# xinxu27/turbo_decoder_cuda

Measured on AMD Instinct MI355X. Metric: decoded info Mbit/s @ K=6144, 8 iter, Eb/N0=1.0 dB; BER match vs CPU log_map, higher is better.
Workload: dtype f64

## Files before the change

include/turbo_mi355x.h:

```cpp
#ifndef TURBO_MI355X_H
#define TURBO_MI355X_H

#include <stdint.h>

#ifdef __cplusplus
extern "C" {
#endif

#define TD_ABI_VERSION 1

enum td_status {
    TD_OK = 0,
    TD_EINVAL = 1,
    TD_ENOMEM = 2,
    TD_EHIP = 3,
    TD_ENODEV = 4
};

enum td_algo {
    TD_ALGO_LOGMAP = 0,
    TD_ALGO_MAXLOG = 1
};

enum td_precision {
// ... 15 lines not shown
int td_create(td_handle** out, const td_params* p);
int td_destroy(td_handle* h);
int td_reserve(td_handle* h, int B);

int td_decode_device(td_handle* h, const void* d_llr, int B, uint8_t* d_bits, int all_iters, void* d_le,
                     void* stream);

int td_debug_window_layout(td_handle* h, int run, int run_a, int parts);
typedef struct td_window_params {
    int window;
    int overlap;
    int nii;
    int concurrent;
    double ext_scale;
} td_window_params;
enum td_window_maxstar { TD_WMAXSTAR_FAST = 0, TD_WMAXSTAR_EXACT = 1 };
int td_set_window_maxstar(td_handle* h, int form);
int td_set_window(td_handle* h, const td_window_params* w);

enum td_stop_rule { TD_STOP_NONE = 0, TD_STOP_HDA = 1, TD_STOP_CRC = 2 };
typedef struct td_stop_params {
    int rule;
    int min_iters;
    uint32_t crc_poly;
} td_stop_params;
int td_set_early_stop(td_handle* h, const td_stop_params* s);
int td_set_window_stop(td_handle* h, const td_stop_params* s);
int td_decode_device_stop(td_handle* h, const void* d_llr, int B, uint8_t* d_bits, int all_iters, void* d_le,
                          int32_t* d_iters, void* stream);
int td_decode_host_stop(td_handle* h, const void* llr, int B, int* out, void* le, int* iters_used);
uint32_t td_crc24_host(const uint8_t* bits, int K, uint32_t poly);
int td_crc24_syndromes(int K, uint32_t poly, uint32_t* table );

int td_profile_enable(td_handle* h, int on);
int td_profile_read(td_handle* h, float* demux_ms, float* decode_ms, int* launches);
int td_clock_read(td_handle* h, double* sclk_ghz, double* span_ms);

int td_debug_set_stamps(td_handle* h, void* d_buf);
int td_debug_stamp_slots(void);
int td_debug_placement(td_handle* h, float* ms, int cap, int* pick);
int td_debug_placement_cost(td_handle* h, double* wall_ms, double* held_bytes);
int td_debug_workspace_bytes(td_handle* h, unsigned long long* bytes);
int td_debug_placement_rule(const float* ms, int n);

int td_window_steps(void);

int td_decode_host(td_handle* h, const void* llr, int B, int* out, void* le);

int td_siso_host(td_handle* h, const void* recs, const void* La, int terminated, void* LLR, int L, int B);

int td_synth_seed(td_handle* h, unsigned seed);
int td_synth_seek(td_handle* h, unsigned long long frame);
int td_rand_window(unsigned seed, unsigned long long draws, uint32_t* win);
int td_synth_frames(td_handle* h, double ebn0_db, int B, uint8_t* d_info, double* d_llr, void* stream);

int td_synth_modulation(td_handle* h, int modulation);

int td_modulate(const uint8_t* d_bits, long long nsym, int modulation, double* d_si, double* d_sq, void* stream);
int td_demodulate(const double* d_yi, const double* d_yq, long long nsym, int modulation, double Kf, double* d_llr,
                  void* stream);

int td_count_errors(td_handle* h, const uint8_t* d_bits, int iters, const uint8_t* d_info, int B, int* d_err,
                    void* stream);

const char* td_last_error(void);
int td_device_count(void);
// ... 14 lines not shown
```

turbo_decoder_cuda_amd/_native.py:

```python
from __future__ import annotations

import ctypes as C
import os

PKG = os.path.dirname(os.path.abspath(__file__))
LIB_PATH = os.environ.get("TD_LIB_PATH") or os.path.join(PKG, "libturbo_mi355x.so")

TD_OK, TD_EINVAL, TD_ENOMEM, TD_EHIP, TD_ENODEV = 0, 1, 2, 3, 4
TD_ALGO_LOGMAP, TD_ALGO_MAXLOG = 0, 1
TD_F64, TD_F32 = 0, 1
TD_WMAXSTAR_FAST, TD_WMAXSTAR_EXACT = 0, 1
TD_MAXSTAR_WINDOW_FAST = 2
TD_STOP_NONE, TD_STOP_HDA, TD_STOP_CRC = 0, 1, 2
CRC24A, CRC24B = 0x864CFB, 0x800063

EXPORTS = (
    "td_create", "td_destroy", "td_reserve", "td_decode_device", "td_decode_host", "td_siso_host",
    "td_last_error", "td_device_count", "td_abi_version", "td_maxstar_host_f64", "td_maxstar_host_f32",
    "td_trellis_tables", "td_qpp_table", "td_profile_enable", "td_profile_read", "td_debug_set_stamps",
    "td_debug_stamp_slots", "td_synth_seed", "td_synth_frames", "td_count_errors", "td_rand_window", "td_synth_seek",
    "td_set_window", "td_synth_modulation", "td_modulate", "td_demodulate", "td_debug_placement",
    "td_debug_placement_rule", "td_clock_read", "td_window_steps", "td_debug_placement_cost", "td_debug_window_layout",
    "td_debug_workspace_bytes", "td_set_window_maxstar", "td_set_early_stop", "td_decode_device_stop",
    "td_decode_host_stop", "td_crc24_host", "td_crc24_syndromes", "td_set_window_stop",
)


class TdParams(C.Structure):
    _fields_ = [
        ("K", C.c_int), ("f1", C.c_int), ("f2", C.c_int), ("iterations", C.c_int),
        ("algo", C.c_int), ("precision", C.c_int), ("device", C.c_int),
    ]


class TdWindowParams(C.Structure):
    _fields_ = [("window", C.c_int), ("overlap", C.c_int), ("nii", C.c_int), ("concurrent", C.c_int),
                ("ext_scale", C.c_double)]


class TdStopParams(C.Structure):
    _fields_ = [("rule", C.c_int), ("min_iters", C.c_int), ("crc_poly", C.c_uint32)]


class TurboError(RuntimeError):
    def __init__(self, code: int, msg: str):
        super().__init__(f"turbo_mi355x error {code}: {msg}")
        self.code = code


_lib = None


def lib() -> C.CDLL:
    global _lib
    if _lib is not None:
        return _lib
    if not os.path.exists(LIB_PATH):
# ... 16 lines not shown
    L.td_device_count.restype = I
    L.td_abi_version.restype = I
    L.td_maxstar_host_f64.argtypes = [C.c_double, C.c_double, I]
    L.td_maxstar_host_f64.restype = C.c_double
    L.td_maxstar_host_f32.argtypes = [C.c_float, C.c_float, I]
    L.td_maxstar_host_f32.restype = C.c_float
    L.td_trellis_tables.argtypes = [P, P, P]
    L.td_qpp_table.argtypes = [I, I, I, P]
    L.td_profile_enable.argtypes = [P, I]
    L.td_debug_set_stamps.argtypes = [P, P]
    L.td_debug_stamp_slots.restype = I
    L.td_debug_placement.argtypes = [P, C.POINTER(C.c_float), I, C.POINTER(C.c_int)]
    L.td_debug_placement_rule.argtypes = [C.POINTER(C.c_float), I]
    if hasattr(L, "td_debug_placement_cost"):
        L.td_debug_placement_cost.argtypes = [P, C.POINTER(C.c_double), C.POINTER(C.c_double)]
    L.td_profile_read.argtypes = [P, C.POINTER(C.c_float), C.POINTER(C.c_float), C.POINTER(C.c_int)]
    if hasattr(L, "td_clock_read"):
        L.td_clock_read.argtypes = [P, C.POINTER(C.c_double), C.POINTER(C.c_double)]
    L.td_synth_seed.argtypes = [P, C.c_uint]
    L.td_rand_window.argtypes = [C.c_uint, C.c_ulonglong, P]
    L.td_synth_seek.argtypes = [P, C.c_ulonglong]
    L.td_synth_frames.argtypes = [P, C.c_double, I, P, P, P]
    L.td_count_errors.argtypes = [P, P, I, P, I, P, P]
    L.td_set_window.argtypes = [P, C.POINTER(TdWindowParams)]
    if hasattr(L, "td_set_early_stop"):
        L.td_set_early_stop.argtypes = [P, C.POINTER(TdStopParams)]
        L.td_decode_device_stop.argtypes = [P, P, I, P, I, P, P, P]
        L.td_decode_host_stop.argtypes = [P, P, I, P, P, P]
        L.td_crc24_host.argtypes = [P, I, C.c_uint32]
        L.td_crc24_host.restype = C.c_uint32
        L.td_crc24_syndromes.argtypes = [I, C.c_uint32, P]
    if hasattr(L, "td_set_window_stop"):
        L.td_set_window_stop.argtypes = [P, C.POINTER(TdStopParams)]
    L.td_synth_modulation.argtypes = [P, I]
    L.td_modulate.argtypes = [P, C.c_longlong, I, P, P, P]
    L.td_demodulate.argtypes = [P, P, C.c_longlong, I, C.c_double, P, P]
    _lib = L
    return L


def check(rc: int) -> None:
    if rc != TD_OK:
        raise TurboError(rc, lib().td_last_error().decode(errors="replace"))
```

turbo_decoder_cuda_amd/csrc/td_api.cpp:

```cpp
#include <hip/hip_runtime_api.h>

#include <cmath>
#include <cstdio>
#include <algorithm>
#include <array>
#include <chrono>
#include <cstdlib>
#include <cstring>
#include <string>
#include <vector>

#include "td_crc.h"
#include "td_kernels.h"

#ifndef TD_SYS2_IN_TURBO
#define TD_SYS2_IN_TURBO 1
#endif
#ifndef TD_PLACEMENT_DEFAULT
#define TD_PLACEMENT_DEFAULT 24
#endif
#include "td_tables.h"
#include "turbo_mi355x.h"

namespace {
// ... 34 lines not shown
    unsigned* d_slots = nullptr;
    unsigned long long* d_clk = nullptr;
    bool clk_valid = false;
    void* d_hin = nullptr;
    uint8_t* d_hbits = nullptr;
    void* d_hle = nullptr;
    size_t hin_b = 0, hbits_b = 0, hle_b = 0;
    int32_t* d_hiters = nullptr;
    size_t hiters_b = 0;
    std::vector<uint8_t> h_hbits;
    void* d_ws = nullptr;
    std::vector<float> place_ms;
    int place_pick = -1;
    double place_wall_ms = 0, place_held = 0;
    size_t ws_bytes = 0;
    size_t elem = 8;
    void* stamps = nullptr;
    bool prof = false;
    std::vector<std::array<hipEvent_t, 3>> ev;
    size_t nev = 0;
    uint32_t lfg_win[31] = {};
    uint32_t lfg_win0[31] = {};
    std::vector<uint32_t> lfg_jump;
    bool lfg_seeded = false;
    unsigned long long lfg_frames = 0;
    uint32_t* d_win = nullptr;
    int win_cap = 0;
    int modulation = 1;
    int role_cus = 0;
    int occ3 = 1;
    td::WindowParams wp{0, 0, 0, 0, 1.0, 0};
    int win_run = 0, win_run_a = 0, win_parts = 0;
    int win_exact_table = 0;
    void* d_wws = nullptr;
    size_t wws_bytes = 0;
    td::WindowStreams wstr{};
    td_stop_params stop{TD_STOP_NONE, 1, 0};
    uint32_t* d_crc = nullptr;
    td_stop_params wstop{TD_STOP_NONE, 1, 0};
    bool clk_stopped = false;
    hipEvent_t ws_free = nullptr;
    hipStream_t ws_stream = nullptr;
    bool ws_pending = false;
};

namespace td {

bool build_lane_tables(const Trellis& t, LaneTables& lt)
{
    auto A = [](int l) { return (l & 1) ^ (((l >> 1) & 1) * 2) ^ (((l >> 2) & 1) * 7); };
    auto rotr = [](int s) { return (s >> 1) | ((s & 1) << 2); };
    const int m[3] = {1, 2, 7};
    for (int ph = 0; ph < 3; ++ph)
        for (int l = 0; l < 8; ++l) {
            int s = A(l);
            for (int r = 0; r < ph; ++r) s = rotr(s);
            lt.state[ph][l] = s;
        }
    for (int ph = 0; ph < 3; ++ph) {
        const int nx = (ph + 1) % 3;
        for (int l = 0; l < 8; ++l) {
            const int j = lt.state[nx][l], ps = lt.state[ph][l], pp = lt.state[ph][l ^ m[ph]];
            const int p0 = t.laststat[j][0], p1 = t.laststat[j][1];
            if (!((ps == p0 && pp == p1) || (ps == p1 && pp == p0))) return false;
            const int us = ps == p0 ? 0 : 1;
            const int os = t.nextout[ps][2 * us + 1], op = t.nextout[pp][2 * (1 - us) + 1];
// ... 333 lines not shown
int decode_device_t(td_handle* h, const void* d_llr, int B, uint8_t* d_bits, int all_iters, void* d_le,
                    int32_t* d_iters, hipStream_t st)
{
    const int G = groups_for(B);
    int rc = ensure_ws(h, G);
    if (rc) return rc;
    const Carve c = carve_for(h, G);
    char* ws = static_cast<char*>(h->d_ws);
    td::DecodeParams<T> dp{};
    fill_common(dp, h);
    dp.sys1 = reinterpret_cast<T*>(ws + c.sys1);
    dp.par1 = reinterpret_cast<T*>(ws + c.par1);
    dp.sys2 = reinterpret_cast<T*>(ws + c.sys2);
    dp.par2 = reinterpret_cast<T*>(ws + c.par2);
    dp.ext12 = reinterpret_cast<T*>(ws + c.ext12);
    dp.ext21 = reinterpret_cast<T*>(ws + c.ext21);
    dp.astore = reinterpret_cast<T*>(ws + c.astore);
    dp.tmstore = reinterpret_cast<T*>(ws + c.tmstore);
    dp.llr_out = nullptr;
    dp.pi = h->d_pi;
    dp.pinv = h->d_pinv;
    dp.bits = d_bits;
    dp.le_dump = static_cast<T*>(d_le);
    dp.stamps = static_cast<unsigned long long*>(h->stamps);
    dp.clk = h->d_clk;
    dp.K = h->p.K;
    dp.L = h->p.K + td::kMemory;
    dp.nT = (dp.L + td::window_steps() - 1) / td::window_steps();
    dp.G = G;
    dp.B = B;
    dp.iters = h->p.iterations;
    dp.all_iters = all_iters ? 1 : 0;
    dp.sys2_in_turbo = (TD_SYS2_IN_TURBO && !h->wp.window) ? 1 : 0;
    td::WindowBufs<T> wb{};
    if (h->wp.window) {
        if (!h->wstr.st[1]) return fail(TD_EINVAL, "td_decode_device: the windowed schedule's streams are missing");
        rc = window_bufs<T>(h, dp, wb);
        if (rc) return rc;
    }
    hipStreamCaptureStatus cap = hipStreamCaptureStatusNone;
    TD_HIP(hipStreamIsCapturing(st, &cap));
    const bool capturing = cap != hipStreamCaptureStatusNone;
    if (!capturing) {
        if (!h->ws_free) TD_HIP(hipEventCreateWithFlags(&h->ws_free, hipEventDisableTiming));
        if (h->ws_pending && st != h->ws_stream) TD_HIP(hipStreamWaitEvent(st, h->ws_free, 0));
    }
    hipEvent_t* ev = nullptr;
    if (h->prof && !capturing) {
        if (h->nev == h->ev.size()) {
            std::array<hipEvent_t, 3> tri{};
            for (auto& x : tri) TD_HIP(hipEventCreate(&x));
            h->ev.push_back(tri);
        }
        ev = h->ev[h->nev].data();
        TD_HIP(hipEventRecord(ev[0], st));
    }
    hipError_t e = h->wp.window ? td::launch_window_demux<T>(dp, static_cast<const T*>(d_llr), st)
                                : td::launch_demux<T>(dp, static_cast<const T*>(d_llr), st);
    if (e != hipSuccess) return hip_fail(e, "launch_demux");
    if (ev) TD_HIP(hipEventRecord(ev[1], st));
    const bool wstop = h->wp.window && h->wstop.rule != TD_STOP_NONE;
    if (wstop) {
        const td::StopParams sp{h->wstop.rule, h->wstop.min_iters, h->d_crc, d_iters};
        e = td::launch_window<T>(dp, h->wp, wb, st, h->wstr, &sp);
    } else if (h->wp.window) {
        e = td::launch_window<T>(dp, h->wp, wb, st, h->wstr);
    } else if (h->stop.rule != TD_STOP_NONE) {
        const td::StopParams sp{h->stop.rule, h->stop.min_iters, h->d_crc, d_iters};
        e = td::launch_turbo<T>(dp, st, false, &sp);
    } else {
        e = td::launch_turbo<T>(dp, st);
    }
    if (e == hipSuccess && d_iters && h->stop.rule == TD_STOP_NONE && !wstop)
        e = hipMemsetD32Async(reinterpret_cast<hipDeviceptr_t>(d_iters), h->p.iterations, (size_t)B, st);
    if (e != hipSuccess) return hip_fail(e, h->wp.window ? "launch_window" : "launch_turbo");
    h->clk_valid = !capturing;
    h->clk_stopped = wstop;
    if (ev) {
        TD_HIP(hipEventRecord(ev[2], st));
        ++h->nev;
    }
    if (!capturing) {
        TD_HIP(hipEventRecord(h->ws_free, st));
        h->ws_stream = st;
        h->ws_pending = true;
    }
    return TD_OK;
}

template <typename T>
int siso_host_t(td_handle* h, const void* recs, const void* La, int terminated, void* LLR, int L, int B)
// ... 399 lines not shown
    const int rc = ensure_wstr(h);
    if (rc) return rc;
    h->wp = td::WindowParams{w->window, w->overlap, w->nii ? 1 : 0, w->concurrent ? 1 : 0, w->ext_scale,
                             h->win_run, h->win_run_a, h->win_parts, h->win_exact_table};
    return TD_OK;
}

int td_set_window_maxstar(td_handle* h, int form)
{
    if (!h) return fail(TD_EINVAL, "td_set_window_maxstar: null handle");
    if (form != TD_WMAXSTAR_FAST && form != TD_WMAXSTAR_EXACT)
        return fail(TD_EINVAL, "td_set_window_maxstar: form must be TD_WMAXSTAR_FAST or TD_WMAXSTAR_EXACT");
    h->win_exact_table = form == TD_WMAXSTAR_EXACT ? 1 : 0;
    h->wp.exact_table = h->win_exact_table;
    return TD_OK;
}

int td_debug_window_layout(td_handle* h, int run, int run_a, int parts)
{
    if (!h) return fail(TD_EINVAL, "td_debug_window_layout: null handle");
    if (run < 0 || run_a < 0 || parts < 0 || parts > td::kSwMaxParts)
        return fail(TD_EINVAL, "td_debug_window_layout: run, run_a >= 0 and 0 <= parts <= 4");
    h->win_run = run;
    h->win_run_a = run_a;
    h->win_parts = parts;
    if (h->wp.window) {
        h->wp.run = run;
        h->wp.run_a = run_a;
        h->wp.parts = parts;
    }
    return TD_OK;
}

int td_profile_enable(td_handle* h, int on)
{
    if (!h) return fail(TD_EINVAL, "td_profile_enable: null handle");
    h->prof = on != 0;
    h->nev = 0;
    return TD_OK;
}

int td_profile_read(td_handle* h, float* demux_ms, float* decode_ms, int* launches)
{
    if (!h || !h->prof) return fail(TD_EINVAL, "td_profile_read: profiling not enabled");
    TD_HIP(hipSetDevice(h->p.device));
    double sa = 0, sb = 0;
    for (size_t k = 0; k < h->nev; ++k) {
        float a = 0, b = 0;
        TD_HIP(hipEventSynchronize(h->ev[k][2]));
        TD_HIP(hipEventElapsedTime(&a, h->ev[k][0], h->ev[k][1]));
        TD_HIP(hipEventElapsedTime(&b, h->ev[k][1], h->ev[k][2]));
        sa += a;
        sb += b;
    }
    const int n = (int)h->nev;
    if (demux_ms) *demux_ms = n ? (float)(sa / n) : 0.f;
    if (decode_ms) *decode_ms = n ? (float)(sb / n) : 0.f;
    if (launches) *launches = n;
    h->nev = 0;
    return TD_OK;
}

int td_clock_read(td_handle* h, double* sclk_ghz, double* span_ms)
{
    if (!h) return fail(TD_EINVAL, "td_clock_read: null handle");
    if (!h->clk_valid) return fail(TD_EINVAL, "td_clock_read: the last decode was captured into a graph");
// ... 220 lines not shown
```

turbo_decoder_cuda_amd/csrc/td_kernels.h:

```cpp
#pragma once

#include <hip/hip_runtime_api.h>

#include <cstdint>

#include "td_tables.h"

namespace td {

struct LaneTables {
    int state[3][8];
    int a_sg[3][8], a_sel[3][8];
    int a_pg[3][8], a_psel[3][8];
    int b_sg[3][8], b_sel[3][8];
    int b_pg[3][8], b_psel[3][8];
    int a_j[3][8];
    int a_swap[3][8];
};

bool build_lane_tables(const Trellis& t, LaneTables& lt);

constexpr int kPermPad = 32;
constexpr int kGroupWaves = 4;
constexpr int kCuSlotKeys = 2048;
constexpr int kWindowStepsMax = 15;
constexpr size_t astore_group_elems(int L) { return ((size_t)L + 1) * 64; }
constexpr size_t astore_elems(int G, int L) { return (size_t)G * astore_group_elems(L) + (size_t)2 * kWindowStepsMax * 64; }

template <typename T>
struct DecodeParams {
    T* sys1;
    T* par1;
    T* sys2;
    T* par2;
    T* ext12;
    T* ext21;
    T* astore;
    T* tmstore;
    T* llr_out;
    const int* pi;
    const int* pinv;
    const LutEntry<T>* lut;
    const T* qlut;
    uint8_t* bits;
    T* le_dump;
    unsigned long long* stamps;
    unsigned long long* clk;
    int K, L, nT, G, B, iters, all_iters, algo;
    int role_cus;
    int occ3;
    int sys2_in_turbo;
    unsigned* cu_slots;
    int nextstat[kStates][2];
    int laststat[kStates][2];
    int nextout[kStates][4];
    const LaneTables* lane;
};

struct StopParams {
    int rule;
    int min_iters;
    const uint32_t* crc_tab;
    int* iters_out;
};

template <typename T>
hipError_t launch_demux(const DecodeParams<T>& p, const T* flow, hipStream_t st);
template <typename T>
hipError_t launch_window_demux(const DecodeParams<T>& p, const T* flow, hipStream_t st);
template <typename T>
hipError_t launch_turbo(const DecodeParams<T>& p, hipStream_t st, bool probe = false,
                        const StopParams* stop = nullptr);
template <typename T, int ALGO>
hipError_t launch_turbo4_w12(const DecodeParams<T>& p, hipStream_t st, const StopParams* stop = nullptr);

struct WindowParams {
    int window;
    int overlap;
    int nii;
    int concurrent;
    double ext_scale;
    int run;
    int run_a;
    int parts;
    int exact_table;
};
template <typename T>
struct WindowBufs {
    T* ext12[2];
    T* ext21[2];
    T* nii;
    T* ckpt[2];
    uint8_t* bitsT;
    int* stop_at;
    unsigned* stop_ev;
};
inline int window_subblocks(int L, int W) { return L / W > 0 ? L / W : 1; }
size_t window_ckpt_elems(int B, int L, int W, bool f32);
// ... 36 lines not shown
```

turbo_decoder_cuda_amd/csrc/td_kernels.hip:

```cpp
#include <hip/hip_runtime.h>

#include <cstdint>
#include <type_traits>

#include "td_kernels.h"
#include "td_tables.h"

#ifdef TD_W12_TU
namespace td_w12 {
using namespace ::td;
#else
namespace td {
#endif

#ifndef TD_KW
#define TD_KW 15
#endif
constexpr int kW = TD_KW;
static_assert(kW == 12 || kW == 15, "windows of 12 or 15 steps");
static_assert(kW <= kWindowStepsMax, "the host sizes the alpha scratch's DMA tail for the longest window");
constexpr int kArow0 = kW / 2;
constexpr int kCw = 8;
constexpr int kLanes = 64;
constexpr int kTile = kW * kCw;
static_assert(kW % 3 == 0, "window must be a multiple of the label period");

#ifndef TD_DIAG
#define TD_DIAG 0
#endif
constexpr unsigned kDiagNoAdma = 1;
constexpr unsigned kDiagNoBConvert = 2;
constexpr unsigned kDiagNoFold = 4;
constexpr unsigned kDiagNoBeta = 8;
constexpr unsigned kDiagOcc3Alias = 16;
constexpr unsigned kDiagNoAStore = 32;
constexpr unsigned kDiagFoldNoLut = 64;
constexpr unsigned kDiagSwNoCk = 128;
// ... 281 lines not shown
{
    if (!kFoldSwz<T>) return off;
    return (off & ~7) + blk_off<T>(off & 7, r);
}

__device__ __forceinline__ void wg_sync_lds()
{
    asm volatile("s_waitcnt lgkmcnt(0)\n\ts_barrier" ::: "memory");
}

template <typename T>
struct SisoSrc {
    const T* sys;
    const T* par;
    const T* la;
    int la_cap;
    int la_len;
    int terminated;
};

template <typename T>
struct SisoDst {
    T* ext;
    int ext_mode;
    int ext_len;
    T* llr;
    T* le_dump;
    uint8_t* bits;
    int bits_row;
    int bits_stride;
    int dump_slot;
    int dump_stride;
    T* sys2_out;
};

struct Geom {
    int K, L, nT, B, g, G;
    const int* pi;
    const int* pinv;
};

__device__ __forceinline__ int window_len(const Geom& gm, int t) { return min(kW, gm.L - t * kW); }

template <typename T>
__device__ __forceinline__ void load_elem(const SisoSrc<T>& src, const Geom& gm, int t, int e, T& ys, T& yp, T& la,
                                          bool want_yp)
{
    const int k = e >> 3, c = e & 7;
    const int i = min(t * kW + k, gm.L - 1);
    const size_t off = ((size_t)gm.g * gm.L + i) * kCw + c;
    ys = src.sys[off];
    yp = want_yp ? src.par[off] : (T)0;
    la = src.la[((size_t)gm.g * src.la_cap + min(i, src.la_cap - 1)) * kCw + c];
}

template <typename T>
__device__ __forceinline__ T la_at(const SisoSrc<T>& src, int i, T raw)
{
    return i < src.la_len ? raw : (T)0;
}

template <int N>
__device__ __forceinline__ void vm_wait()
{
    asm volatile("s_waitcnt vmcnt(%0)" ::"n"(N) : "memory");
}
// ... 984 lines not shown
        asm volatile("s_waitcnt lgkmcnt(0)" ::: "memory");
        TD_STAMP(bc);
        TD_ACC(14, b0, bc);
        tile_dma(sm, slot, src, dst, gm, max(min(wa - 3, tl - 3), 0), lane);
        tm_dma(sm, slot, tmstore, gm, wa - 3, lane);
        if constexpr (kAd > 0) alpha_dma<T, ALGO>(sm, astore, gm, wa - 1, lane);
        TD_STAMP(bw);
        vm_wait<2 * kB>();
        TD_STAMP(b1);
        TD_ACC(4, bw, b1);
        wg_sync_lds();
        TD_STAMP(b2);
        TD_ACC(2, b0, b1);
        TD_ACC(3, b1, b2);
    };
    tile_dma(sm, 0, src, dst, gm, max(tl - 3, 0), lane);
    tm_dma(sm, 0, tmstore, gm, tl, lane);
    tile_dma(sm, 1, src, dst, gm, max(tl - 3, 0), lane);
    tm_dma(sm, 1, tmstore, gm, tl - 1, lane);
    tile_dma(sm, 2, src, dst, gm, max(tl - 3, 0), lane);
    tm_dma(sm, 2, tmstore, gm, tl - 2, lane);
    if constexpr (kAd > 0) alpha_dma<T, ALGO>(sm, astore, gm, tl, lane);
    vm_wait<2 * (kF + 1) + kAd>();
    TD_STAMP(p4);
    TD_ACC(12, p3, p4);
    for (int j = 0; j < nB; j += 3) {
        bstep(j, 0);
        if (j + 1 < nB) bstep(j + 1, 1);
        if (j + 2 < nB) bstep(j + 2, 2);
    }
    asm volatile("s_waitcnt vmcnt(0)" ::: "memory");
}

template <typename T, int ALGO, bool STOP = false>
__device__ void siso_wg(Smem<T>& sm, const SisoSrc<T>& src, const SisoDst<T>& dst, const Geom& gm, T* astore,
                        T* tmstore, const LaneTables* lt, int wave, int lane, unsigned long long* st,
                        StopLane* sl = nullptr)
{
    (void)st;
    (void)sl;
    if constexpr (kRoleRemat<T>) touch(lane);
    TD_STAMP(p0);
    const int nT = gm.nT;
    const int tl = nT - 1;
    const int nB = nT + 2;
    T* ga0 = astore + astore_window_off(gm.g, 0, gm.L);
    constexpr size_t aws = (size_t)kW * kLanes;
    T* gtm0 = tmstore + (size_t)gm.g * gm.L * kCw;

    if (wave == 0) {
        const int c = lane >> 3;
        LaneConst<T> lc;
        lane_setup(lt, lane, lc);
        T a = lc.a_init0 ? (T)0 : (T)-kInfty;
        __builtin_amdgcn_s_setprio(kAlphaPrio);
        wg_sync_lds();
        TD_STAMP(p1);
        TD_ACC(11, p0, p1);
        int t0 = 0;
        if constexpr (kAlphaSchedS<T, ALGO>) {
            if (tl >= 2) {
                TD_STAMP(f0);
                a = alpha_window<T, ALGO>(a, 0, kW, sm, lut_col(sm, lane), c, lc, ga0, gtm0, st ? st + 4 : nullptr);
                TD_STAMP(f1);
                wg_sync_lds();
                TD_STAMP(f2);
                TD_ACC(0, f0, f1);
                TD_ACC(1, f1, f2);
// ... 61 lines not shown
    } else if (wave == 2) {
        constexpr int kF = kTileDma<T>;
        auto fstep = [&](int t) {
            TD_STAMP(f0);
            if (t + 1 <= tl) tile_convert(sm, (t + 1) % 3, src, t + 1, lane);
            if (!kFSkip<ALGO> || t + 3 <= tl) {
                tile_dma(sm, t % 3, src, dst, gm, min(t + 3, tl), lane);
                vm_wait<kF>();
            } else {
                vm_wait<0>();
            }
            TD_STAMP(f1);
            wg_sync_lds();
            TD_STAMP(f2);
            TD_ACC(0, f0, f1);
            TD_ACC(1, f1, f2);
        };
        tile_dma(sm, 0, src, dst, gm, 0, lane);
        vm_wait<0>();
        TD_STAMP(p2);
        TD_ACC(13, p0, p2);
        tile_convert(sm, 0, src, 0, lane);
        tile_dma(sm, 1, src, dst, gm, min(1, tl), lane);
        tile_dma(sm, 2, src, dst, gm, min(2, tl), lane);
        vm_wait<kF>();
        wg_sync_lds();
        TD_STAMP(p1);
        TD_ACC(11, p0, p1);
        for (int t = 0; t < nT; ++t) fstep(t);
        if constexpr (kBLoaderWave<ALGO> == 2) {
            bpass_loader<T, ALGO>(sm, src, dst, gm, astore, tmstore, lane, tl, nB, st);
            return;
        }
    } else if (dst.sys2_out) {
        wg_sync_lds();
        TD_STAMP(p1);
        TD_ACC(11, p0, p1);
        const int e = (wave == 1 ? 0 : kLanes) + lane;
        const int ec = min(e, kTile - 1);
        const int k = ec >> 3, c = ec & 7;
        const T* s1 = src.sys + (size_t)gm.g * gm.L * kCw + c;
        T* s2 = dst.sys2_out + (size_t)gm.g * gm.L * kCw + c;
        T v = (T)0;
        int ip = -1;
        for (int t = 0; t < nT; ++t) {
            TD_STAMP(f0);
            const int pi_i = min(max(sm.Wp[t % 3][k][1], 0), gm.K - 1);
            const T nv = s1[(size_t)pi_i * kCw];
            if (ip >= 0) s2[(size_t)ip * kCw] = v;
            const int i = t * kW + k;
            ip = (e < kTile && i < gm.K) ? i : -1;
            v = nv;
            TD_STAMP(f1);
            wg_sync_lds();
            TD_STAMP(f2);
            TD_ACC(0, f0, f1);
            TD_ACC(1, f1, f2);
        }
        if (ip >= 0) s2[(size_t)ip * kCw] = v;
        asm volatile("s_waitcnt vmcnt(0)" ::: "memory");
    } else {
        wg_sync_lds();
        TD_STAMP(p1);
        TD_ACC(11, p0, p1);
        for (int t = 0; t < nT; ++t) {
            TD_STAMP(f0);
// ... 213 lines not shown
__device__ __forceinline__ void wg_release(const WgPos& w, unsigned* slots)
{
    if (w.slot < 4) {
        __syncthreads();
        if (threadIdx.x == 0) atomicAnd(&slots[w.slot_key], ~(1u << w.slot));
    }
}

template <typename T, int ALGO, bool STOP = false>
__device__ __forceinline__ void turbo_decode_body(const DecodeParams<T>& p, const StopParams* sp = nullptr)
{
    (void)sp;
    const WgPos w = wg_pos(p.role_cus, p.cu_slots);
    Smem<T>& sm = *smem<T>();
    const int wave = w.role, lane = w.lane;
    lut_to_lds(p, sm, wave * kLanes + lane);
    if (wave == 1) set_beta_prio<T, ALGO>();
    [[maybe_unused]] StopLane sl{};
    [[maybe_unused]] unsigned long long used = 0;
    [[maybe_unused]] int stop_first = 0;
    if constexpr (STOP) {
        __shared__ unsigned s_stop[kCw];
        if (threadIdx.x < kCw) s_stop[threadIdx.x] = 0;
        sl.rule = sp->rule;
        sl.crc_tab = sp->crc_tab;
        sl.lds = s_stop;
        sl.prev_off = p.all_iters ? -(long long)p.K : 0;
        for (int c = 0; c < kCw; ++c) {
            if (w.g * kCw + c >= p.B) sl.done |= 1u << c;
            used |= (unsigned long long)p.iters << (8 * c);
        }
        stop_first = max(sp->rule == 1 ? 2 : 1, sp->min_iters);
    }
    __syncthreads();

    Geom gm{p.K, p.L, p.nT, p.B, w.g, p.G, p.pi, p.pinv};
    unsigned long long st[kStampSlots] = {};
#ifdef TD_STAMPS
    const unsigned long long k_cyc0 = __builtin_amdgcn_s_memtime(), k_rt0 = __builtin_amdgcn_s_memrealtime();
#endif
    const bool clk = p.clk && blockIdx.x == 0;
    unsigned long long clk_c0 = 0, clk_r0 = 0;
    if (clk) {
        clk_c0 = __builtin_amdgcn_s_memtime();
        clk_r0 = __builtin_amdgcn_s_memrealtime();
    }
    for (int s = 0; s < 2 * p.iters; ++s) {
        const int it = s >> 1, dec = s & 1;
        const bool want_bits = dec == 1 && (STOP || p.all_iters || it == p.iters - 1);
        SisoSrc<T> src{dec ? p.sys2 : p.sys1, dec ? p.par2 : p.par1, dec ? p.ext12 : p.ext21, p.K,
                       (dec == 0 && it == 0) ? 0 : p.K, 1};
        SisoDst<T> dst{dec ? p.ext21 : p.ext12, dec ? 2 : 3, p.K, nullptr, p.le_dump,
                       want_bits ? p.bits : nullptr, p.all_iters ? it : 0, p.all_iters ? p.iters * p.K : p.K,
                       s, p.iters * 2 * p.L, (s == 0 && p.sys2_in_turbo) ? p.sys2 : nullptr};
        TD_STAMP(s0);
        if constexpr (STOP) {
            sl.acc = 0;
            sl.has_prev = it > 0;
        }
        siso_wg<T, ALGO, STOP>(sm, src, dst, gm, p.astore, p.tmstore, p.lane, wave, lane, st, &sl);
        TD_STAMP(s1);
        __syncthreads();
        TD_STAMP(s2);
        TD_ACC(9, s0, s1);
        TD_ACC(10, s1, s2);
        if constexpr (STOP) {
            if (dec == 1 && it + 1 < p.iters) {
                unsigned stop = 0;
                if (it + 1 >= stop_first) {
                    if (sl.rule == 1) {
                        stop = ~sl.lds[0] & 0xffu;
                    } else {
#pragma unroll
                        for (int c = 0; c < kCw; ++c) stop |= (sl.lds[c] == 0 ? 1u : 0u) << c;
                    }
                }
                stop = (unsigned)__builtin_amdgcn_readfirstlane((int)stop) & ~sl.done;
#pragma unroll
                for (int c = 0; c < kCw; ++c)
                    if ((stop >> c) & 1)
                        used = (used & ~(0xffull << (8 * c))) | ((unsigned long long)(it + 1) << (8 * c));
                sl.done |= stop;
                __syncthreads();
                if (threadIdx.x < kCw) sl.lds[threadIdx.x] = 0;
                if (sl.done == 0xffu) break;
            }
        }
// ... 949 lines not shown
    if (e != hipSuccess) return e;
    if (probe)
        hipLaunchKernelGGL((turbo_placement_probe_kernel<T, ALGO>), dim3(p.G), dim3(kWaves * kLanes), wg_lds<T>(), st, p);
    else
        hipLaunchKernelGGL((turbo_decode_kernel<T, ALGO>), dim3(p.G), dim3(kWaves * kLanes), wg_lds<T>(), st, p);
    return hipGetLastError();
}

template <typename T, int ALGO>
hipError_t launch_siso_algo(const DecodeParams<T>& p, const T* la, int terminated, hipStream_t st)
{
    hipError_t e = allow_smem(reinterpret_cast<const void*>(&siso_kernel<T, ALGO>), wg_lds<T>());
    if (e != hipSuccess) return e;
    hipLaunchKernelGGL((siso_kernel<T, ALGO>), dim3(p.G), dim3(kWaves * kLanes), wg_lds<T>(), st, p, la, terminated);
    return hipGetLastError();
}

template <typename T>
hipError_t launch_demux(const DecodeParams<T>& p, const T* flow, hipStream_t st)
{
    const size_t total = (size_t)p.G * p.L * kCw;
    int gblocks = (int)((total + 255) / 256);
    if (gblocks > kDemuxBlocks) gblocks = kDemuxBlocks;
    hipLaunchKernelGGL(demux_kernel<T>, dim3(gblocks), dim3(256), 0, st, p, flow);
    hipError_t e = hipGetLastError();
    if (e != hipSuccess) return e;
    if (p.sys2_in_turbo) return hipSuccess;
    const int bpg = (p.K * kCw + kPermBlock - 1) / kPermBlock;
    const long long pblocks = (long long)((p.G + 7) / 8) * 8 * bpg;
    hipLaunchKernelGGL(demux_perm_kernel<T>, dim3((unsigned)pblocks), dim3(kPermBlock), 0, st, p, bpg);
    return hipGetLastError();
}

template <typename T>
hipError_t launch_turbo(const DecodeParams<T>& p, hipStream_t st, bool probe, const StopParams* stop)
{
    return p.algo == 1 ? launch_turbo_algo<T, 1>(p, st, probe, stop) : launch_turbo_algo<T, 0>(p, st, probe, stop);
}

template <typename T>
hipError_t launch_siso(const DecodeParams<T>& p, const T* recs, const T* la, T* la_ws, int terminated, T* llr,
                       hipStream_t st)
{
    const size_t total = (size_t)p.G * p.L * kCw;
    int gblocks = (int)((total + 255) / 256);
    if (gblocks > kDemuxBlocks) gblocks = kDemuxBlocks;
    hipLaunchKernelGGL(siso_in_kernel<T>, dim3(gblocks), dim3(256), 0, st, p, recs, la, la_ws);
    hipError_t e = p.algo == 1 ? launch_siso_algo<T, 1>(p, la_ws, terminated, st)
                               : launch_siso_algo<T, 0>(p, la_ws, terminated, st);
    if (e != hipSuccess) return e;
    hipLaunchKernelGGL(siso_out_kernel<T>, dim3(gblocks), dim3(256), 0, st, p, llr);
    return hipGetLastError();
}

#if !defined(TD_W12_TU) && !defined(TD_WIN_TU)
template hipError_t launch_demux<double>(const DecodeParams<double>&, const double*, hipStream_t);
template hipError_t launch_demux<float>(const DecodeParams<float>&, const float*, hipStream_t);
template hipError_t launch_turbo<double>(const DecodeParams<double>&, hipStream_t, bool, const StopParams*);
template hipError_t launch_turbo<float>(const DecodeParams<float>&, hipStream_t, bool, const StopParams*);
template hipError_t launch_siso<double>(const DecodeParams<double>&, const double*, const double*, double*, int,
                                        double*, hipStream_t);
template hipError_t launch_siso<float>(const DecodeParams<float>&, const float*, const float*, float*, int, float*,
                                       hipStream_t);

int window_steps() { return kW; }
#endif
#ifdef TD_WIN_TU
template hipError_t launch_window_demux<double>(const DecodeParams<double>&, const double*, hipStream_t);
template hipError_t launch_window_demux<float>(const DecodeParams<float>&, const float*, hipStream_t);
template hipError_t launch_window<double>(const DecodeParams<double>&, const WindowParams&, const WindowBufs<double>&,
                                         hipStream_t, const WindowStreams&, const StopParams*);
template hipError_t launch_window<float>(const DecodeParams<float>&, const WindowParams&, const WindowBufs<float>&,
                                        hipStream_t, const WindowStreams&, const StopParams*);
#endif

}

#ifdef TD_W12_TU
namespace td {
template <typename T, int ALGO>
hipError_t launch_turbo4_w12(const DecodeParams<T>& p, hipStream_t st, const StopParams* stop)
{
    static_assert(td_w12::kOcc4<T, ALGO>, "the 12-step-window build has the four-per-CU kernel");
    DecodeParams<T> q = p;
    q.nT = (q.L + td_w12::kW - 1) / td_w12::kW;
    return td_w12::launch_kernel4<T, ALGO>(q, st, stop);
}
template hipError_t launch_turbo4_w12<float, 0>(const DecodeParams<float>&, hipStream_t, const StopParams*);
template hipError_t launch_turbo4_w12<float, 1>(const DecodeParams<float>&, hipStream_t, const StopParams*);
}
// ... 2 lines not shown
```

turbo_decoder_cuda_amd/decoder.py:

```python
from __future__ import annotations

import ctypes as C

import numpy as np

from . import _native as N

N_ITERATION = 15
TERMINATED = 1

_ALGOS = {"logmap": N.TD_ALGO_LOGMAP, "maxlog": N.TD_ALGO_MAXLOG}
_PRECS = {"f64": N.TD_F64, "f32": N.TD_F32}
_STOP_RULES = {None: N.TD_STOP_NONE, "hda": N.TD_STOP_HDA, "crc": N.TD_STOP_CRC}


def stream_length(K: int) -> int:
    return 3 * K + 12


class TurboCodec:
    def __init__(self, K: int, f1: int, f2: int, iterations: int = N_ITERATION, algo: str = "logmap",
                 precision: str = "f64", device: int = 0):
        self.K, self.f1, self.f2 = int(K), int(f1), int(f2)
        self.L = self.K + 3
# ... 47 lines not shown
    def workspace_bytes(self) -> int:
        v = C.c_ulonglong(0)
        N.check(N.lib().td_debug_workspace_bytes(self._h, C.byref(v)))
        return int(v.value)

    def set_window_maxstar(self, exact: bool) -> None:
        N.check(N.lib().td_set_window_maxstar(self._h, N.TD_WMAXSTAR_EXACT if exact else N.TD_WMAXSTAR_FAST))

    def set_window(self, window: int = 64, overlap: int = 30, ext_scale: float = 1.0, nii: bool = False,
                   concurrent: bool = False) -> None:
        w = N.TdWindowParams(int(window), int(overlap), int(bool(nii)), int(bool(concurrent)), float(ext_scale))
        N.check(N.lib().td_set_window(self._h, C.byref(w)))
        self.window = int(window)
        if not self.window and self._window_stop:
            self.early_stop, self._window_stop = None, False

    def set_early_stop(self, rule=None, min_iters: int = 1, crc_poly: int = N.CRC24B) -> None:
        if rule not in _STOP_RULES:
            raise ValueError(f"rule must be 'hda', 'crc' or None, got {rule!r}")
        s = N.TdStopParams(_STOP_RULES[rule], int(min_iters), int(crc_poly) & 0xFFFFFFFF)
        N.check(N.lib().td_set_early_stop(self._h, C.byref(s)))
        self.early_stop = rule

    def set_window_early_stop(self, rule=None, min_iters: int = 1, crc_poly: int = N.CRC24B) -> None:
        if rule not in _STOP_RULES:
            raise ValueError(f"rule must be 'hda', 'crc' or None, got {rule!r}")
        s = N.TdStopParams(_STOP_RULES[rule], int(min_iters), int(crc_poly) & 0xFFFFFFFF)
        N.check(N.lib().td_set_window_stop(self._h, C.byref(s)))
        self.early_stop = rule
        self._window_stop = rule is not None

    def debug_window_layout(self, run: int = 0, run_a: int = 0, parts: int = 0) -> None:
        N.check(N.lib().td_debug_window_layout(self._h, int(run), int(run_a), int(parts)))

    def TurboDecoding(self, flow: np.ndarray, return_le: bool = False, return_iters: bool = False):
        flow = np.ascontiguousarray(flow, dtype=self.dtype)
        one = flow.ndim == 1
        flow = flow.reshape(-1, stream_length(self.K))
        B = flow.shape[0]
        out = np.zeros((B, self.iterations, self.K), dtype=np.int32)
        le = np.zeros((B, self.iterations, 2, self.L), dtype=self.dtype) if return_le else None
        used = np.zeros(B, dtype=np.int32) if return_iters else None
        le_p = le.ctypes.data_as(C.c_void_p) if return_le else None
        if return_iters:
            N.check(N.lib().td_decode_host_stop(self._h, flow.ctypes.data_as(C.c_void_p), B,
                                                out.ctypes.data_as(C.c_void_p), le_p, used.ctypes.data_as(C.c_void_p)))
        else:
            N.check(N.lib().td_decode_host(self._h, flow.ctypes.data_as(C.c_void_p), B,
                                           out.ctypes.data_as(C.c_void_p), le_p))
        if one:
            out, le = out[0], (le[0] if return_le else None)
            used = int(used[0]) if return_iters else None
        res = (out,) + ((le,) if return_le else ()) + ((used,) if return_iters else ())
        return res if len(res) > 1 else out

    def decode(self, llr, bits=None, all_iters: bool = False, le=None, stream=None, iters_out=None):
        import torch

        want = torch.float64 if self.precision == "f64" else torch.float32
        if llr.dtype != want or not llr.is_cuda or not llr.is_contiguous():
            raise ValueError(f"llr must be a contiguous {want} CUDA tensor")
        if llr.ndim != 2 or llr.shape[1] != stream_length(self.K):
            raise ValueError(f"llr must be [B, {stream_length(self.K)}] (3K+12), got {tuple(llr.shape)}")
        if llr.device.index != self.device:
            raise ValueError(f"llr is on {llr.device}, the codec on cuda:{self.device}")
        B = llr.shape[0]
# ... 137 lines not shown
```

Baseline: 1544.

## Fuse demux into the turbo kernel's first SISO pass

Removes the separate demux kernel launch for f64 non-windowed decoding. The turbo kernel now demuxes the first windows up front and then streams the remaining windows of the LLR flow into the sys1/par1/par2/sys2 buffers during the first half-iteration. These loads are interleaved with the forward pass on idle waves under a lead/period schedule. This saves a launch and a full global round trip before decoding starts, at the cost of extra work and register pressure inside the first SISO pass and a forced inline of siso_wg.

```diff
diff --git a/include/turbo_mi355x.h b/include/turbo_mi355x.h
--- a/include/turbo_mi355x.h
+++ b/include/turbo_mi355x.h
@@ -71,6 +71,9 @@
 uint32_t td_crc24_host(const uint8_t* bits, int K, uint32_t poly);
 int td_crc24_syndromes(int K, uint32_t poly, uint32_t* table );
 
+int td_debug_demux_fused(td_handle* h, int mode);
+int td_debug_demux_path(td_handle* h, int* fused);
+
 int td_profile_enable(td_handle* h, int on);
 int td_profile_read(td_handle* h, float* demux_ms, float* decode_ms, int* launches);
 int td_clock_read(td_handle* h, double* sclk_ghz, double* span_ms);
diff --git a/turbo_decoder_cuda_amd/_native.py b/turbo_decoder_cuda_amd/_native.py
--- a/turbo_decoder_cuda_amd/_native.py
+++ b/turbo_decoder_cuda_amd/_native.py
@@ -22,7 +22,8 @@
     "td_set_window", "td_synth_modulation", "td_modulate", "td_demodulate", "td_debug_placement",
     "td_debug_placement_rule", "td_clock_read", "td_window_steps", "td_debug_placement_cost", "td_debug_window_layout",
     "td_debug_workspace_bytes", "td_set_window_maxstar", "td_set_early_stop", "td_decode_device_stop",
-    "td_decode_host_stop", "td_crc24_host", "td_crc24_syndromes", "td_set_window_stop",
+    "td_decode_host_stop", "td_crc24_host", "td_crc24_syndromes", "td_set_window_stop", "td_debug_demux_fused",
+    "td_debug_demux_path",
 )
 
 
@@ -105,6 +106,9 @@
         L.td_crc24_syndromes.argtypes = [I, C.c_uint32, P]
     if hasattr(L, "td_set_window_stop"):
         L.td_set_window_stop.argtypes = [P, C.POINTER(TdStopParams)]
+    if hasattr(L, "td_debug_demux_fused"):
+        L.td_debug_demux_fused.argtypes = [P, I]
+        L.td_debug_demux_path.argtypes = [P, C.POINTER(C.c_int)]
     L.td_synth_modulation.argtypes = [P, I]
     L.td_modulate.argtypes = [P, C.c_longlong, I, P, P, P]
     L.td_demodulate.argtypes = [P, P, C.c_longlong, I, C.c_double, P, P]
diff --git a/turbo_decoder_cuda_amd/csrc/td_api.cpp b/turbo_decoder_cuda_amd/csrc/td_api.cpp
--- a/turbo_decoder_cuda_amd/csrc/td_api.cpp
+++ b/turbo_decoder_cuda_amd/csrc/td_api.cpp
@@ -90,6 +90,8 @@
     td::WindowParams wp{0, 0, 0, 0, 1.0, 0};
     int win_run = 0, win_run_a = 0, win_parts = 0;
     int win_exact_table = 0;
+    int demux_mode = 1;
+    int demux_last = -1;
     void* d_wws = nullptr;
     size_t wws_bytes = 0;
     td::WindowStreams wstr{};
@@ -489,6 +491,13 @@
     dp.iters = h->p.iterations;
     dp.all_iters = all_iters ? 1 : 0;
     dp.sys2_in_turbo = (TD_SYS2_IN_TURBO && !h->wp.window) ? 1 : 0;
+    dp.flow = static_cast<const T*>(d_llr);
+    dp.demux_in_turbo = (h->demux_mode && dp.sys2_in_turbo && !h->wp.window &&
+                         (3 * (size_t)dp.K + 4 * td::kMemory) * sizeof(T) % 16 == 0 &&
+                         reinterpret_cast<uintptr_t>(d_llr) % 16 == 0 && td::demux_fused_built<T>(dp))
+                            ? 1
+                            : 0;
+    h->demux_last = dp.demux_in_turbo;
     td::WindowBufs<T> wb{};
     if (h->wp.window) {
         if (!h->wstr.st[1]) return fail(TD_EINVAL, "td_decode_device: the windowed schedule's streams are missing");
@@ -512,8 +521,11 @@
         ev = h->ev[h->nev].data();
         TD_HIP(hipEventRecord(ev[0], st));
     }
-    hipError_t e = h->wp.window ? td::launch_window_demux<T>(dp, static_cast<const T*>(d_llr), st)
-                                : td::launch_demux<T>(dp, static_cast<const T*>(d_llr), st);
+    hipError_t e = hipSuccess;
+    if (h->wp.window)
+        e = td::launch_window_demux<T>(dp, static_cast<const T*>(d_llr), st);
+    else if (!dp.demux_in_turbo)
+        e = td::launch_demux<T>(dp, static_cast<const T*>(d_llr), st);
     if (e != hipSuccess) return hip_fail(e, "launch_demux");
     if (ev) TD_HIP(hipEventRecord(ev[1], st));
     const bool wstop = h->wp.window && h->wstop.rule != TD_STOP_NONE;
@@ -979,6 +991,21 @@
     return TD_OK;
 }
 
+int td_debug_demux_fused(td_handle* h, int mode)
+{
+    if (!h) return fail(TD_EINVAL, "td_debug_demux_fused: null handle");
+    if (mode != 0 && mode != 1) return fail(TD_EINVAL, "td_debug_demux_fused: mode must be 0 or 1");
+    h->demux_mode = mode;
+    return TD_OK;
+}
+
+int td_debug_demux_path(td_handle* h, int* fused)
+{
+    if (!h || !fused) return fail(TD_EINVAL, "td_debug_demux_path: null argument");
+    *fused = h->demux_last;
+    return TD_OK;
+}
+
 int td_profile_enable(td_handle* h, int on)
 {
     if (!h) return fail(TD_EINVAL, "td_profile_enable: null handle");
diff --git a/turbo_decoder_cuda_amd/csrc/td_demux_addr.h b/turbo_decoder_cuda_amd/csrc/td_demux_addr.h
--- /dev/null
+++ b/turbo_decoder_cuda_amd/csrc/td_demux_addr.h
@@ -0,0 +1,54 @@
+#pragma once
+
+#if defined(__HIPCC__) || defined(__CUDACC__)
+#define TD_HD __host__ __device__
+#else
+#define TD_HD
+#endif
+
+namespace td {
+
+constexpr int kDemuxTail = 3;
+constexpr int kDemuxPeriod = 4;
+constexpr int kDemuxTurn = 2;
+constexpr int kDemuxLead = 9;
+static_assert(kDemuxTurn * 2 == kDemuxPeriod, "two waves, each kDemuxTurn windows a turn, cover every window");
+static_assert(kDemuxLead - 4 >= kDemuxPeriod + 1, "a window is complete and published before the loader reads it");
+TD_HD inline bool demux_active(int q, int t) { return t % kDemuxPeriod == kDemuxTurn * q; }
+
+enum DemuxField { kDmSys1 = 0, kDmPar1 = 1, kDmPar2 = 2, kDmSys2 = 3 };
+
+TD_HD inline int demux_src(int K, int i, int f)
+{
+    if (i < K) return 3 * i + (f == kDmSys2 ? 0 : f);
+    const int j = i - K;
+    const int t1 = 3 * K + 2 * j, t2 = 3 * K + 2 * kDemuxTail + 2 * j;
+    return f == kDmSys1 ? t1 : f == kDmPar1 ? t1 + 1 : f == kDmSys2 ? t2 : t2 + 1;
+}
+
+struct DemuxItem {
+    int i;
+    int c;
+    bool real;
+};
+TD_HD inline DemuxItem demux_item(int K, int kw, int w, int e)
+{
+    const int L = K + kDemuxTail, tile = kw * 8;
+    const int tl = (L + kw - 1) / kw - 1;
+    const int ec = e < tile ? e : tile - 1;
+    const int iu = w * kw + (ec >> 3);
+    const int wc = w < tl ? w : tl;
+    int i = wc * kw + (ec >> 3);
+    if (i > L - 1) i = L - 1;
+    return DemuxItem{i, ec & 7, w <= tl && e < tile && iu < L};
+}
+
+TD_HD inline int demux_sys2_row(int K, int i, int pinv_i)
+{
+    if (i >= K) return i;
+    return pinv_i < 0 ? 0 : (pinv_i > K - 1 ? K - 1 : pinv_i);
+}
+
+TD_HD inline int demux_src_row(int B, int b) { return b < B ? b : B - 1; }
+
+}
diff --git a/turbo_decoder_cuda_amd/csrc/td_kernels.h b/turbo_decoder_cuda_amd/csrc/td_kernels.h
--- a/turbo_decoder_cuda_amd/csrc/td_kernels.h
+++ b/turbo_decoder_cuda_amd/csrc/td_kernels.h
@@ -55,6 +55,8 @@
     int laststat[kStates][2];
     int nextout[kStates][4];
     const LaneTables* lane;
+    const T* flow;
+    int demux_in_turbo;
 };
 
 struct StopParams {
@@ -64,6 +66,8 @@
     int* iters_out;
 };
 
+template <typename T>
+bool demux_fused_built(const DecodeParams<T>& p);
 template <typename T>
 hipError_t launch_demux(const DecodeParams<T>& p, const T* flow, hipStream_t st);
 template <typename T>
diff --git a/turbo_decoder_cuda_amd/csrc/td_kernels.hip b/turbo_decoder_cuda_amd/csrc/td_kernels.hip
--- a/turbo_decoder_cuda_amd/csrc/td_kernels.hip
+++ b/turbo_decoder_cuda_amd/csrc/td_kernels.hip
@@ -3,6 +3,7 @@
 #include <cstdint>
 #include <type_traits>
 
+#include "td_demux_addr.h"
 #include "td_kernels.h"
 #include "td_tables.h"
 
@@ -350,6 +351,8 @@
     int dump_slot;
     int dump_stride;
     T* sys2_out;
+    const T* flow;
+    T* par2_out;
 };
 
 struct Geom {
@@ -1400,8 +1403,89 @@
     asm volatile("s_waitcnt vmcnt(0)" ::: "memory");
 }
 
+#ifdef TD_STAMPS
+constexpr bool kDemuxBuild = false;
+#else
+constexpr bool kDemuxBuild = kW == 15;
+#endif
+template <typename T, int ALGO>
+constexpr bool kDemuxFused = kDemuxBuild && sizeof(T) == 8;
+static_assert(kDemuxTail == kMemory, "td_demux_addr.h's tail steps");
+static_assert(kMemory + 1 <= kPermPad, "pinv is read at the clamped tail steps");
+
+template <typename T>
+struct DemuxVals {
+    T v[4];
+    int s2row;
+};
+template <typename T>
+__device__ __forceinline__ DemuxVals<T> demux_load(const T* flow, const Geom& gm, int i, int c)
+{
+    const int b = gm.g * kCw + c;
+    const T* r = flow + (size_t)demux_src_row(gm.B, b) * (size_t)(3 * gm.K + 4 * kMemory);
+    DemuxVals<T> d;
+#pragma unroll
+    for (int f = 0; f < 4; ++f) {
+        const T x = r[demux_src(gm.K, i, f)] * (T)0.5;
+        d.v[f] = b < gm.B ? x : (T)0;
+    }
+    d.s2row = demux_sys2_row(gm.K, i, gm.pinv[i]);
+    return d;
+}
+template <typename T>
+struct DemuxOut {
+    T *sys1, *par1, *par2, *sys2;
+};
+template <typename T>
+__device__ __forceinline__ void demux_store(const DemuxOut<T>& o, const Geom& gm, int i, int c, const DemuxVals<T>& d)
+{
+    const size_t g0 = (size_t)gm.g * gm.L, e = (g0 + i) * kCw + c;
+    o.sys1[e] = d.v[kDmSys1];
+    o.par1[e] = d.v[kDmPar1];
+    o.par2[e] = d.v[kDmPar2];
+    o.sys2[(g0 + d.s2row) * kCw + c] = d.v[kDmSys2];
+}
+template <typename T>
+__device__ __forceinline__ void demux_head(const DemuxOut<T>& o, const T* flow, const Geom& gm)
+{
+    const int n = min(kDemuxLead * kW, gm.L) * kCw;
+    for (int e = (int)threadIdx.x; e < n; e += kWaves * kLanes)
+        demux_store(o, gm, e >> 3, e & 7, demux_load(flow, gm, e >> 3, e & 7));
+    vm_wait<0>();
+}
+template <typename T>
+__device__ __forceinline__ void demux_fpass(const DemuxOut<T>& o, const T* flow, const Geom& gm, int q, int lane, int nT)
+{
+    static_assert(kDemuxTurn == 2, "four named items per lane");
+    DemuxVals<T> d0, d1, d2, d3;
+    DemuxItem i0, i1, i2, i3;
+#define TD_DEMUX_LOAD(ix, dx, w, e)          \
+    ix = demux_item(gm.K, kW, (w), (e));     \
+    dx = demux_load(flow, gm, ix.i, ix.c)
+#define TD_DEMUX_LOAD_TURN(w0)                      \
+    TD_DEMUX_LOAD(i0, d0, (w0), lane);              \
+    TD_DEMUX_LOAD(i1, d1, (w0), lane + kLanes);     \
+    TD_DEMUX_LOAD(i2, d2, (w0) + 1, lane);          \
+    TD_DEMUX_LOAD(i3, d3, (w0) + 1, lane + kLanes)
+    TD_DEMUX_LOAD_TURN(kDemuxLead + kDemuxTurn * q);
+    for (int t = 0; t < nT; ++t) {
+        if (demux_active(q, t)) {
+            vm_wait<0>();
+            if (i0.real) demux_store(o, gm, i0.i, i0.c, d0);
+            if (i1.real) demux_store(o, gm, i1.i, i1.c, d1);
+            if (i2.real) demux_store(o, gm, i2.i, i2.c, d2);
+            if (i3.real) demux_store(o, gm, i3.i, i3.c, d3);
+            TD_DEMUX_LOAD_TURN(t + kDemuxPeriod + kDemuxLead);
+        }
+        wg_sync_lds();
+    }
+#undef TD_DEMUX_LOAD_TURN
+#undef TD_DEMUX_LOAD
+    vm_wait<0>();
+}
+
 template <typename T, int ALGO, bool STOP = false>
-__device__ void siso_wg(Smem<T>& sm, const SisoSrc<T>& src, const SisoDst<T>& dst, const Geom& gm, T* astore,
+__device__ __forceinline__ void siso_wg(Smem<T>& sm, const SisoSrc<T>& src, const SisoDst<T>& dst, const Geom& gm, T* astore,
                         T* tmstore, const LaneTables* lt, int wave, int lane, unsigned long long* st,
                         StopLane* sl = nullptr)
 {
@@ -1529,6 +1613,12 @@
             bpass_loader<T, ALGO>(sm, src, dst, gm, astore, tmstore, lane, tl, nB, st);
             return;
         }
+    } else if (kDemuxFused<T, ALGO> && dst.flow) {
+        wg_sync_lds();
+        TD_STAMP(p1);
+        TD_ACC(11, p0, p1);
+        demux_fpass(DemuxOut<T>{const_cast<T*>(src.sys), const_cast<T*>(src.par), dst.par2_out, dst.sys2_out}, dst.flow, gm,
+                    wave == 1 ? 0 : 1, lane, nT);
     } else if (dst.sys2_out) {
         wg_sync_lds();
         TD_STAMP(p1);
@@ -1808,9 +1898,14 @@
         }
         stop_first = max(sp->rule == 1 ? 2 : 1, sp->min_iters);
     }
+    Geom gm{p.K, p.L, p.nT, p.B, w.g, p.G, p.pi, p.pinv};
+    bool demux = false;
+    if constexpr (kDemuxFused<T, ALGO>) {
+        demux = p.demux_in_turbo && p.sys2_in_turbo && p.flow;
+        if (demux) demux_head(DemuxOut<T>{p.sys1, p.par1, p.par2, p.sys2}, p.flow, gm);
+    }
     __syncthreads();
 
-    Geom gm{p.K, p.L, p.nT, p.B, w.g, p.G, p.pi, p.pinv};
     unsigned long long st[kStampSlots] = {};
 #ifdef TD_STAMPS
     const unsigned long long k_cyc0 = __builtin_amdgcn_s_memtime(), k_rt0 = __builtin_amdgcn_s_memrealtime();
@@ -1828,7 +1923,8 @@
                        (dec == 0 && it == 0) ? 0 : p.K, 1};
         SisoDst<T> dst{dec ? p.ext21 : p.ext12, dec ? 2 : 3, p.K, nullptr, p.le_dump,
                        want_bits ? p.bits : nullptr, p.all_iters ? it : 0, p.all_iters ? p.iters * p.K : p.K,
-                       s, p.iters * 2 * p.L, (s == 0 && p.sys2_in_turbo) ? p.sys2 : nullptr};
+                       s, p.iters * 2 * p.L, (s == 0 && p.sys2_in_turbo) ? p.sys2 : nullptr,
+                       (s == 0 && demux) ? p.flow : nullptr, p.par2};
         TD_STAMP(s0);
         if constexpr (STOP) {
             sl.acc = 0;
@@ -2844,6 +2940,18 @@
     return hipGetLastError();
 }
 
+template <typename T, int ALGO>
+bool demux_fused_algo(const DecodeParams<T>& p)
+{
+    if (occupancy_pick<T, ALGO>(p) == 4 && !kOcc4<T, ALGO>) return false;
+    return kDemuxFused<T, ALGO>;
+}
+template <typename T>
+bool demux_fused_built(const DecodeParams<T>& p)
+{
+    return p.algo == 1 ? demux_fused_algo<T, 1>(p) : demux_fused_algo<T, 0>(p);
+}
+
 template <typename T>
 hipError_t launch_turbo(const DecodeParams<T>& p, hipStream_t st, bool probe, const StopParams* stop)
 {
@@ -2868,6 +2976,8 @@
 #if !defined(TD_W12_TU) && !defined(TD_WIN_TU)
 template hipError_t launch_demux<double>(const DecodeParams<double>&, const double*, hipStream_t);
 template hipError_t launch_demux<float>(const DecodeParams<float>&, const float*, hipStream_t);
+template bool demux_fused_built<double>(const DecodeParams<double>&);
+template bool demux_fused_built<float>(const DecodeParams<float>&);
 template hipError_t launch_turbo<double>(const DecodeParams<double>&, hipStream_t, bool, const StopParams*);
 template hipError_t launch_turbo<float>(const DecodeParams<float>&, hipStream_t, bool, const StopParams*);
 template hipError_t launch_siso<double>(const DecodeParams<double>&, const double*, const double*, double*, int,
diff --git a/turbo_decoder_cuda_amd/decoder.py b/turbo_decoder_cuda_amd/decoder.py
--- a/turbo_decoder_cuda_amd/decoder.py
+++ b/turbo_decoder_cuda_amd/decoder.py
@@ -103,6 +103,14 @@
 
     def debug_window_layout(self, run: int = 0, run_a: int = 0, parts: int = 0) -> None:
         N.check(N.lib().td_debug_window_layout(self._h, int(run), int(run_a), int(parts)))
+
+    def debug_demux_fused(self, on: bool = True) -> None:
+        N.check(N.lib().td_debug_demux_fused(self._h, int(bool(on))))
+
+    def demux_path(self) -> int:
+        v = C.c_int(-1)
+        N.check(N.lib().td_debug_demux_path(self._h, C.byref(v)))
+        return int(v.value)
 
     def TurboDecoding(self, flow: np.ndarray, return_le: bool = False, return_iters: bool = False):
         flow = np.ascontiguousarray(flow, dtype=self.dtype)
```

New measurement: 1546, median of 6. About the same (+0.2%).
